# veeresht/CommPy

Measured on AMD Instinct MI355X. Metric: decoded info-bits/s at fixed Eb/N0 (Viterbi K=7 r=1/2, 1024b); BER match, higher is better.
Workload: dtype f64

## Files before the change

commpy_amd/csrc/viterbi_cw.hip:

```cpp
#include "cpx_internal.h"
#include "cpx_math.h"
#include "viterbi_cw_asm.h"
#ifndef CPX_GEN_GB
#define CPX_GEN_GB 2
#endif

#include <atomic>
#include <cstdlib>
#include <cstring>
#include <mutex>
#include <type_traits>

using namespace cpx;

namespace {

template <int LGS, unsigned G0, unsigned G1>
struct SrCode {
    static constexpr int S = 1 << LGS;
    static constexpr int parity(unsigned v) { return __builtin_popcount(v) & 1; }
    static constexpr int code(int s, int j) {
        const unsigned p = (unsigned)(((s << 1) & (S - 1)) | j), b = (unsigned)(s >> (LGS - 1));
        const unsigned reg = (b << LGS) | p;
        return (parity(reg & G0) << 1) | parity(reg & G1);
    }
};

template <int LGS>
constexpr int rotl(int s, int r) {
    r %= LGS;
    return r == 0 ? s : (((s << r) | (s >> (LGS - r))) & ((1 << LGS) - 1));
}

__device__ __forceinline__ double vmin(double a, double b) {
    double r;
    asm("v_min_f64 %0, %1, %2" : "=v"(r) : "v"(a), "v"(b));
    return r;
}

__device__ __forceinline__ double acs_min(unsigned &acc, double x, double y) {
    double r;
    asm("v_cmp_lt_f64 vcc, %3, %2\n\tv_addc_co_u32 %1, vcc, %1, %1, vcc\n\tv_min_f64 %0, %2, %3"
        : "=&v"(r), "+v"(acc) : "v"(x), "v"(y) : "vcc");
    return r;
}
__device__ __forceinline__ double acs_min_first(unsigned &acc, double x, double y) {
    double r;
    asm("v_cmp_lt_f64 vcc, %3, %2\n\tv_cndmask_b32 %1, 0, 1, vcc\n\tv_min_f64 %0, %2, %3"
        : "=&v"(r), "=&v"(acc) : "v"(x), "v"(y) : "vcc");
    return r;
}

__device__ __forceinline__ double acs_select(unsigned &acc, double x, double y) {
    int rlo, rhi;
    asm("v_cmp_lt_f64 vcc, %4, %3\n\tv_cndmask_b32 %0, %5, %7, vcc\n\tv_cndmask_b32 %1, %6, %8, vcc\n\t"
        "v_addc_co_u32 %2, vcc, %2, %2, vcc"
        : "=&v"(rlo), "=&v"(rhi), "+v"(acc)
        : "v"(x), "v"(y), "v"(__double2loint(x)), "v"(__double2hiint(x)), "v"(__double2loint(y)), "v"(__double2hiint(y))
        : "vcc");
    return __hiloint2double(rhi, rlo);
}

struct CwParams {
    const double *coded;
    unsigned long long *dec;
    unsigned char *best;
    uint8_t *bits;
    uint8_t *nanflags;
    int64_t B, len, L, T, Lk, Tp;
    int type, tb;
    unsigned goff[4];
};

__device__ __forceinline__ void nan_or(unsigned long long &mask, double r0, double r1) {
#ifdef CPX_AB_NO_NAN_DETECT
    (void)mask; (void)r0; (void)r1;
    return;
#endif
    asm("v_cmp_u_f64 vcc, %1, %2\n\ts_or_b64 %0, %0, vcc" : "+s"(mask) : "v"(r0), "v"(r1) : "vcc", "scc");
}

__device__ __forceinline__ void bit_metrics_cw(int type, double r, double &m0, double &m1) {
    if (type == CPX_VIT_HARD) {
        long long ri = (long long)r;
        m0 = (double)(ri ^ 0ll);
        m1 = (double)(ri ^ 1ll);
    } else if (type == CPX_VIT_SOFT) {
        double nll0 = fast_log<false>(exp(r) + 1.0);
        m0 = nll0;
        m1 = nll0 - r;
    } else {
        double d0 = r - (-1.0), d1 = r - 1.0;
        m0 = d0 * d0;
        m1 = d1 * d1;
    }
}

__device__ __forceinline__ double clip500(double r) {
    double c;
    asm("v_max_f64 %0, %1, %2\n\tv_min_f64 %0, %0, %3" : "=&v"(c) : "v"(r), "s"(-500.0), "s"(500.0));
    return c;
}
__device__ __forceinline__ void soft_metrics_lean(double r, double &m0, double &m1) {
    const double nll0 = fast_log<false, false, true>(exp_pm500(r) + 1.0);
    m0 = nll0;
    m1 = nll0 - r;
}

template <int LGS>
__device__ __forceinline__ unsigned tb_hop(unsigned long long w, unsigned st) {
    const unsigned hi = (unsigned)((w << (st & ((1u << LGS) - 1u))) >> 32);
    return __builtin_amdgcn_alignbit(st, hi, 31);
}

struct NoHook {
    template <int P> __device__ __forceinline__ void at() const {}
};

template <int LGS, unsigned G0, unsigned G1, int TYPE, int R, bool LEAN = false, class Hook = NoHook>
__device__ __forceinline__ void cw_step(double (&pm)[1 << LGS], double r0, double r1, unsigned long long &word, int &best,
                                        const Hook &hook = Hook(), unsigned char *bml = nullptr, const unsigned *gidx = nullptr) {
    constexpr int type = TYPE;
    using C = SrCode<LGS, G0, G1>;
    constexpr bool GEN = G0 == 0 && G1 == 0;
    constexpr int S = 1 << LGS, H = S / 2;
    double m00, m01, m10, m11;
    if constexpr (LEAN && TYPE == CPX_VIT_SOFT) {
        r0 = clip500(r0);
        r1 = clip500(r1);
        soft_metrics_lean(r0, m00, m01);
        soft_metrics_lean(r1, m10, m11);
    } else {
        if (type == CPX_VIT_SOFT) {
            r0 = fmin(fmax(r0, -500.0), 500.0);
            r1 = fmin(fmax(r1, -500.0), 500.0);
        }
        bit_metrics_cw(type, r0, m00, m01);
        bit_metrics_cw(type, r1, m10, m11);
    }
    double bmv[4];
    if constexpr (LEAN) {
        bmv[0] = m00 + m10; bmv[1] = m00 + m11;
        bmv[2] = m01 + m10; bmv[3] = m01 + m11;
    } else {
        bmv[0] = (0.0 + m00) + m10; bmv[1] = (0.0 + m00) + m11;
        bmv[2] = (0.0 + m01) + m10; bmv[3] = (0.0 + m01) + m11;
    }
    unsigned da = 0, db = 0;
    hook.template at<0>();
    auto butterfly = [&](int j, double m_a0, double m_a1, double m_b0, double m_b1) {
        const int x = rotl<LGS>(2 * j, R), y = rotl<LGS>(2 * j + 1, R);
        const double a = pm[x], b = pm[y];
        const double a0 = a + m_a0, a1 = b + m_a1;
        const double b0 = a + m_b0, b1 = b + m_b1;
        if (TYPE == CPX_VIT_UNQUANTIZED) {
            pm[x] = acs_select(da, a0, a1);
            pm[y] = acs_select(db, b0, b1);
        } else if (j == 0) {
            pm[x] = acs_min_first(da, a0, a1);
            pm[y] = acs_min_first(db, b0, b1);
        } else {
            pm[x] = acs_min(da, a0, a1);
            pm[y] = acs_min(db, b0, b1);
        }
    };
    if constexpr (GEN) {
        typedef double cpx_d4 __attribute__((ext_vector_type(4)));
        const cpx_d4 tab = {bmv[0], bmv[1], bmv[2], bmv[3]}, rtab = {bmv[3], bmv[2], bmv[1], bmv[0]};
        asm volatile("s_set_gpr_idx_on 0, 1" ::: "memory", "m0");
        auto acs_pair = [&](int j, double a0, double a1, double b0, double b1) {
            const int x = rotl<LGS>(2 * j, R), y = rotl<LGS>(2 * j + 1, R);
            if (TYPE == CPX_VIT_UNQUANTIZED) {
                pm[x] = acs_select(da, a0, a1);
                pm[y] = acs_select(db, b0, b1);
            } else {
                pm[x] = acs_min(da, a0, a1);
                pm[y] = acs_min(db, b0, b1);
            }
        };
        if constexpr (H >= 4 && TYPE != CPX_VIT_UNQUANTIZED) {
#pragma unroll
            for (int j = 0; j < H; j += 2) {
                if (j == H / 2) hook.template at<1>();
                const int x0 = rotl<LGS>(2 * j, R), y0 = rotl<LGS>(2 * j + 1, R), x1 = rotl<LGS>(2 * j + 2, R), y1 = rotl<LGS>(2 * j + 3, R);
                const double a = pm[x0], b = pm[y0], c = pm[x1], d = pm[y1];
                double a0, a1, b0, b1, c0, c1, d0, d1;
                asm volatile("s_set_gpr_idx_idx %[i0]\n\t"
                             "v_add_f64 %[a0], v[248:249], %[a]\n\t"
                             "v_add_f64 %[b1], v[248:249], %[b]\n\t"
                             "v_add_f64 %[a1], v[240:241], %[b]\n\t"
                             "v_add_f64 %[b0], v[240:241], %[a]\n\t"
                             "s_set_gpr_idx_idx %[i1]\n\t"
                             "v_add_f64 %[c0], v[248:249], %[c]\n\t"
                             "v_add_f64 %[d1], v[248:249], %[d]\n\t"
                             "v_add_f64 %[c1], v[240:241], %[d]\n\t"
                             "v_add_f64 %[d0], v[240:241], %[c]\n\t"
                             "s_set_gpr_idx_idx 0\n\t"
                             "v_cmp_lt_f64 vcc, %[a1], %[a0]\n\tv_addc_co_u32 %[da], vcc, %[da], %[da], vcc\n\tv_min_f64 %[a0], %[a0], %[a1]\n\t"
                             "v_cmp_lt_f64 vcc, %[b1], %[b0]\n\tv_addc_co_u32 %[db], vcc, %[db], %[db], vcc\n\tv_min_f64 %[b0], %[b0], %[b1]\n\t"
                             "v_cmp_lt_f64 vcc, %[c1], %[c0]\n\tv_addc_co_u32 %[da], vcc, %[da], %[da], vcc\n\tv_min_f64 %[c0], %[c0], %[c1]\n\t"
                             "v_cmp_lt_f64 vcc, %[d1], %[d0]\n\tv_addc_co_u32 %[db], vcc, %[db], %[db], vcc\n\tv_min_f64 %[d0], %[d0], %[d1]"
                             : [a0] "=&v"(a0), [a1] "=&v"(a1), [b0] "=&v"(b0), [b1] "=&v"(b1), [c0] "=&v"(c0), [c1] "=&v"(c1),
                               [d0] "=&v"(d0), [d1] "=&v"(d1), [da] "+v"(da), [db] "+v"(db)
                             : [i0] "s"(gidx[j]), [i1] "s"(gidx[j + 1]), [a] "v"(a), [b] "v"(b), [c] "v"(c), [d] "v"(d),
                               "{v[248:255]}"(tab), "{v[240:247]}"(rtab)
                             : "vcc", "m0");
                pm[x0] = a0; pm[y0] = b0;
                pm[x1] = c0; pm[y1] = d0;
            }
        } else {
#pragma unroll
            for (int j = 0; j < H; j++) {
                if (j == H / 2) hook.template at<1>();
                const double a = pm[rotl<LGS>(2 * j, R)], b = pm[rotl<LGS>(2 * j + 1, R)];
                double a0, a1, b0, b1;
                asm volatile("s_set_gpr_idx_idx %[ic]\n\t"
                             "v_add_f64 %[a0], v[248:249], %[a]\n\t"
                             "v_add_f64 %[b1], v[248:249], %[b]\n\t"
                             "v_add_f64 %[a1], v[240:241], %[b]\n\t"
                             "v_add_f64 %[b0], v[240:241], %[a]\n\t"
                             "s_set_gpr_idx_idx 0"
                             : [a0] "=&v"(a0), [a1] "=&v"(a1), [b0] "=&v"(b0), [b1] "=&v"(b1)
                             : [ic] "s"(gidx[j]), [a] "v"(a), [b] "v"(b), "{v[248:255]}"(tab), "{v[240:247]}"(rtab)
                             : "m0");
                acs_pair(j, a0, a1, b0, b1);
            }
        }
        asm volatile("s_set_gpr_idx_off" ::: "memory", "m0");
    } else {
#pragma unroll
        for (int j = 0; j < H; j++) {
            if (j == H / 2) hook.template at<1>();
            butterfly(j, bmv[C::code(j, 0)], bmv[C::code(j, 1)], bmv[C::code(j + H, 0)], bmv[C::code(j + H, 1)]);
        }
    }
    hook.template at<2>();
    int bst = 0;
    constexpr bool ARGMIN32 = LEAN && S == 64 && TYPE == CPX_VIT_SOFT && !GEN;
    unsigned long long tie = ~0ull;
    if constexpr (ARGMIN32) {
#define CPX_HI(s) "v"(__double2hiint(pm[rotl<LGS>((s), R + 1)]))
#define CPX_COL(i) CPX_HI(i), CPX_HI((i) + 8), CPX_HI((i) + 16), CPX_HI((i) + 24), CPX_HI((i) + 32), CPX_HI((i) + 40), CPX_HI((i) + 48), CPX_HI((i) + 56)
#define CPX_ROW(j) CPX_HI(8 * (j)), CPX_HI(8 * (j) + 1), CPX_HI(8 * (j) + 2), CPX_HI(8 * (j) + 3), CPX_HI(8 * (j) + 4), CPX_HI(8 * (j) + 5), CPX_HI(8 * (j) + 6), CPX_HI(8 * (j) + 7)
        unsigned q0, q1, q2, q3, q4, q5, q6, q7, m, w;
        asm(CPX_COL_BLOCK3 : "=&v"(q0), "=&v"(q1), "=&v"(q2) : CPX_COL(0), CPX_COL(1), CPX_COL(2));
        asm(CPX_COL_BLOCK3 : "=&v"(q3), "=&v"(q4), "=&v"(q5) : CPX_COL(3), CPX_COL(4), CPX_COL(5));
        asm(CPX_COL_BLOCK_LAST : "=&v"(q6), "=&v"(q7), "=&v"(m), "=&v"(w) : "v"(q0), "v"(q1), "v"(q2), "v"(q3), "v"(q4), "v"(q5), CPX_COL(6), CPX_COL(7)
            : "vcc");
        hook.template at<3>();
        unsigned r0_, r1_, r2_;
        asm(CPX_ROW_BLOCK3 : "+v"(w), "=&v"(r0_), "=&v"(r1_), "=&v"(r2_) : "v"(m), CPX_ROW(7), CPX_ROW(6), CPX_ROW(5) : "vcc");
        asm(CPX_ROW_BLOCK3 : "+v"(w), "=&v"(r0_), "=&v"(r1_), "=&v"(r2_) : "v"(m), CPX_ROW(4), CPX_ROW(3), CPX_ROW(2) : "vcc");
        asm(CPX_ROW_BLOCK_LAST : "+v"(w), "=&v"(r0_), "=&v"(r1_), "=&v"(bst), "=&s"(tie) : "v"(m), CPX_ROW(1), CPX_ROW(0) : "vcc");
#undef CPX_ROW
#undef CPX_COL
#undef CPX_HI
    }
    if (__builtin_expect(tie != 0, !ARGMIN32)) {
        double m0 = pm[0], m1 = pm[1 % S], m2 = pm[2 % S], m3 = pm[3 % S];
        if constexpr (S == 64) {
#define CPX_V4(a) "v"(pm[a]), "v"(pm[(a) + 1]), "v"(pm[(a) + 2]), "v"(pm[(a) + 3])
            asm(CPX_MIN_BLOCK24 : "+v"(m0), "+v"(m1), "+v"(m2), "+v"(m3)
                : CPX_V4(4), CPX_V4(8), CPX_V4(12), CPX_V4(16), CPX_V4(20), CPX_V4(24));
            asm(CPX_MIN_BLOCK24 : "+v"(m0), "+v"(m1), "+v"(m2), "+v"(m3)
                : CPX_V4(28), CPX_V4(32), CPX_V4(36), CPX_V4(40), CPX_V4(44), CPX_V4(48));
            asm(CPX_MIN_BLOCK12 : "+v"(m0), "+v"(m1), "+v"(m2), "+v"(m3) : CPX_V4(52), CPX_V4(56), CPX_V4(60));
#undef CPX_V4
        } else {
#pragma unroll
            for (int s = 4; s < S; s += 4) {
                m0 = vmin(m0, pm[s]); m1 = vmin(m1, pm[s + 1]); m2 = vmin(m2, pm[s + 2]); m3 = vmin(m3, pm[s + 3]);
            }
        }
        const double mn = vmin(vmin(m0, m1), vmin(m2, m3));
        if constexpr (!ARGMIN32) hook.template at<3>();
        if constexpr (S == 64) {
            unsigned long long k0, k1, k2, k3;
#define CPX_S4(a) "v"(pm[rotl<LGS>((a), R + 1)]), "v"(pm[rotl<LGS>((a) - 1, R + 1)]), "v"(pm[rotl<LGS>((a) - 2, R + 1)]), "v"(pm[rotl<LGS>((a) - 3, R + 1)])
            asm(CPX_SCAN_BLOCK0 : "+v"(bst), "=&s"(k0), "=&s"(k1), "=&s"(k2), "=&s"(k3)
                : "v"(mn), CPX_S4(63), CPX_S4(59), CPX_S4(55), CPX_S4(51), CPX_S4(47), CPX_S4(43));
            asm(CPX_SCAN_BLOCK1 : "+v"(bst), "=&s"(k0), "=&s"(k1), "=&s"(k2), "=&s"(k3)
                : "v"(mn), CPX_S4(39), CPX_S4(35), CPX_S4(31), CPX_S4(27), CPX_S4(23), CPX_S4(19));
            asm(CPX_SCAN_BLOCK2 : "+v"(bst), "=&s"(k0), "=&s"(k1), "=&s"(k2), "=&s"(k3)
                : "v"(mn), CPX_S4(15), CPX_S4(11), CPX_S4(7), CPX_S4(3));
#undef CPX_S4
        } else if constexpr (S % 4 == 0) {
#pragma unroll
            for (int s = S - 4; s >= 0; s -= 4) {
                unsigned long long k0, k1, k2, k3;
                asm("v_cmp_eq_f64 %1, %5, %9\n\tv_cmp_eq_f64 %2, %6, %9\n\tv_cmp_eq_f64 %3, %7, %9\n\tv_cmp_eq_f64 %4, %8, %9\n\t"
                    "v_cndmask_b32 %0, %0, %10, %1\n\tv_cndmask_b32 %0, %0, %11, %2\n\tv_cndmask_b32 %0, %0, %12, %3\n\t"
                    "v_cndmask_b32 %0, %0, %13, %4"
                    : "+v"(bst), "=&s"(k0), "=&s"(k1), "=&s"(k2), "=&s"(k3)
                    : "v"(pm[rotl<LGS>(s + 3, R + 1)]), "v"(pm[rotl<LGS>(s + 2, R + 1)]), "v"(pm[rotl<LGS>(s + 1, R + 1)]),
                      "v"(pm[rotl<LGS>(s, R + 1)]), "v"(mn), "n"(s + 3), "n"(s + 2), "n"(s + 1), "n"(s));
            }
        } else {
#pragma unroll
            for (int s = S - 1; s >= 0; s--) bst = (pm[rotl<LGS>(s, R + 1)] == mn) ? s : bst;
        }
    }
    word = ((unsigned long long)da << (64 - H)) | ((unsigned long long)db << (64 - S));
    best = bst;
}

__device__ __forceinline__ float acs_min_f32(unsigned &acc, float x, float y) {
    float r;
    asm("v_cmp_lt_f32 vcc, %3, %2\n\tv_addc_co_u32 %1, vcc, %1, %1, vcc\n\tv_min_f32 %0, %2, %3"
        : "=&v"(r), "+v"(acc) : "v"(x), "v"(y) : "vcc");
    return r;
}
__device__ __forceinline__ float vmin3_f32(float a, float b, float c) {
    float r;
    asm("v_min3_f32 %0, %1, %2, %3" : "=v"(r) : "v"(a), "v"(b), "v"(c));
    return r;
}
__device__ __forceinline__ void bit_metrics_f32(int type, double r, float &m0, float &m1) {
    if (type == CPX_VIT_HARD) {
        const long long ri = (long long)r;
        m0 = (float)(ri ^ 0ll);
        m1 = (float)(ri ^ 1ll);
    } else if (type == CPX_VIT_SOFT) {
        m0 = 0.0f;
        m1 = -(float)r;
    } else {
        const float x = (float)r, d0 = x + 1.0f, d1 = x - 1.0f;
        m0 = d0 * d0;
        m1 = d1 * d1;
    }
}

template <int LGS, unsigned G0, unsigned G1, int TYPE, int R, bool LEAN = false, class Hook = NoHook>
__device__ __forceinline__ void cw_step(float (&pm)[1 << LGS], double r0, double r1, unsigned long long &word, int &best,
                                        const Hook &hook = Hook(), unsigned char * = nullptr, const unsigned * = nullptr) {
    using C = SrCode<LGS, G0, G1>;
    constexpr int S = 1 << LGS, H = S / 2;
    if (TYPE == CPX_VIT_SOFT) {
        r0 = fmin(fmax(r0, -500.0), 500.0);
        r1 = fmin(fmax(r1, -500.0), 500.0);
    }
    float m00, m01, m10, m11;
    bit_metrics_f32(TYPE, r0, m00, m01);
    bit_metrics_f32(TYPE, r1, m10, m11);
    float bmv[4];
    bmv[0] = (0.0f + m00) + m10; bmv[1] = (0.0f + m00) + m11;
    bmv[2] = (0.0f + m01) + m10; bmv[3] = (0.0f + m01) + m11;
    unsigned da = 0, db = 0;
    hook.template at<0>();
#pragma unroll
    for (int j = 0; j < H; j++) {
        if (j == H / 2) hook.template at<1>();
        const int x = rotl<LGS>(2 * j, R), y = rotl<LGS>(2 * j + 1, R);
        const float a = pm[x], b = pm[y];
        const float a0 = a + bmv[C::code(j, 0)], a1 = b + bmv[C::code(j, 1)];
        const float b0 = a + bmv[C::code(j + H, 0)], b1 = b + bmv[C::code(j + H, 1)];
        pm[x] = acs_min_f32(da, a0, a1);
        pm[y] = acs_min_f32(db, b0, b1);
    }
    hook.template at<2>();
    float mn;
    if constexpr (S >= 8 && S % 8 == 0) {
        float m0 = pm[0], m1 = pm[1], m2 = pm[2], m3 = pm[3];
#pragma unroll
        for (int s = 4; s + 8 <= S; s += 8) {
            m0 = vmin3_f32(m0, pm[s], pm[s + 1]); m1 = vmin3_f32(m1, pm[s + 2], pm[s + 3]);
            m2 = vmin3_f32(m2, pm[s + 4], pm[s + 5]); m3 = vmin3_f32(m3, pm[s + 6], pm[s + 7]);
        }
        m0 = vmin3_f32(m0, pm[S - 4], pm[S - 3]);
        m1 = vmin3_f32(m1, pm[S - 2], pm[S - 1]);
        mn = fminf(vmin3_f32(m0, m1, m2), m3);
    } else {
        mn = pm[0];
#pragma unroll
        for (int s = 1; s < S; s++) mn = fminf(mn, pm[s]);
    }
    hook.template at<3>();
    int bst = 0;
    if constexpr (S % 4 == 0) {
#pragma unroll
        for (int s = S - 4; s >= 0; s -= 4) {
            unsigned long long k0, k1, k2, k3;
            asm("v_cmp_eq_f32 %1, %5, %9\n\tv_cmp_eq_f32 %2, %6, %9\n\tv_cmp_eq_f32 %3, %7, %9\n\tv_cmp_eq_f32 %4, %8, %9\n\t"
                "v_cndmask_b32 %0, %0, %10, %1\n\tv_cndmask_b32 %0, %0, %11, %2\n\tv_cndmask_b32 %0, %0, %12, %3\n\t"
                "v_cndmask_b32 %0, %0, %13, %4"
                : "+v"(bst), "=&s"(k0), "=&s"(k1), "=&s"(k2), "=&s"(k3)
                : "v"(pm[rotl<LGS>(s + 3, R + 1)]), "v"(pm[rotl<LGS>(s + 2, R + 1)]), "v"(pm[rotl<LGS>(s + 1, R + 1)]),
                  "v"(pm[rotl<LGS>(s, R + 1)]), "v"(mn), "n"(s + 3), "n"(s + 2), "n"(s + 1), "n"(s));
        }
    } else {
#pragma unroll
        for (int s = S - 1; s >= 0; s--) bst = (pm[rotl<LGS>(s, R + 1)] == mn) ? s : bst;
    }
    word = ((unsigned long long)da << (64 - H)) | ((unsigned long long)db << (64 - S));
    best = bst;
}

constexpr int ACS_WAVES = 4;

template <int LGS, unsigned G0, unsigned G1, int TYPE>
__global__ __launch_bounds__(64 * ACS_WAVES) void viterbi_cw_acs_kernel(CwParams p) {
    constexpr int S = 1 << LGS;
    const int lane = threadIdx.x & 63;
    const int64_t grp = (int64_t)blockIdx.x * ACS_WAVES + (threadIdx.x >> 6);
    const int64_t cw = grp * 64 + lane;
    if (grp * 64 >= p.B) return;
    const bool valid = cw < p.B;
    const double *x = p.coded + (valid ? cw : 0) * p.len;
    unsigned long long *dec = p.dec + grp * p.Tp * 64 + lane;
    unsigned char *best = p.best + grp * p.Tp * 64 + lane;

    double pm[S];
#pragma unroll
    for (int s = 0; s < S; s++) pm[s] = (s == 0) ? 0.0 : __builtin_huge_val();

    const double pad = (TYPE == CPX_VIT_UNQUANTIZED) ? -1.0 : 0.0;
    const int T = (int)p.T, tmax = (int)((p.Lk < p.T) ? p.Lk : p.T);
    auto load = [&](int t) {
        const int tc = (t < tmax) ? t : tmax;
        return *reinterpret_cast<const double2 *>(x + (int64_t)(tc - 1) * 2);
    };
    double2 cur[LGS], nxt[LGS];
#pragma unroll
    for (int u = 0; u < LGS; u++) cur[u] = load(1 + u);
    unsigned long long nanmask = 0;
    for (int t = 1; t <= T; t += LGS) {
#pragma unroll
        for (int u = 0; u < LGS; u++) nxt[u] = load(t + LGS + u);
#pragma unroll
        for (int u = 0; u < LGS; u++) {
            const bool have = t + u <= tmax;
            cur[u].x = have ? cur[u].x : pad;
            cur[u].y = have ? cur[u].y : pad;
        }
        unsigned long long *d = dec + (int64_t)(t - 1) * 64;
        unsigned char *b = best + (int64_t)(t - 1) * 64;
        auto one = [&](auto rtag, const double2 &v) {
            constexpr int R = decltype(rtag)::value;
            unsigned long long word;
            int bst;
            if constexpr (TYPE == CPX_VIT_SOFT) nan_or(nanmask, v.x, v.y);
            cw_step<LGS, G0, G1, TYPE, R>(pm, v.x, v.y, word, bst);
            d[R * 64] = word;
            b[R * 64] = (unsigned char)bst;
        };
        if constexpr (LGS >= 1) one(std::integral_constant<int, 0>{}, cur[0]);
        if constexpr (LGS >= 2) one(std::integral_constant<int, 1>{}, cur[1 % LGS]);
        if constexpr (LGS >= 3) one(std::integral_constant<int, 2>{}, cur[2 % LGS]);
        if constexpr (LGS >= 4) one(std::integral_constant<int, 3>{}, cur[3 % LGS]);
        if constexpr (LGS >= 5) one(std::integral_constant<int, 4>{}, cur[4 % LGS]);
        if constexpr (LGS >= 6) one(std::integral_constant<int, 5>{}, cur[5 % LGS]);
#pragma unroll
        for (int u = 0; u < LGS; u++) cur[u] = nxt[u];
    }
    static_assert(LGS == 6, "viterbi_cw_acs_kernel writes per-codeword NaN flags: valid for 64-state trellises only (items of one codeword)");
    if constexpr (TYPE == CPX_VIT_SOFT)
        if (valid) p.nanflags[cw] = (uint8_t)((nanmask >> lane) & 1ull);
}

constexpr int FR_RING = 32, FR_CHUNK = 96, FR_OBPAD = 100;
constexpr int FR_RING_DEEP = 64;

template <int RING, bool MIR> constexpr int fused_slots() { return MIR ? 2 * RING + 2 : RING + 1; }
template <int RING, bool MIR, bool GEN = false>
constexpr size_t fused_wave_lds() {
    return (size_t)fused_slots<RING, MIR>() * 64 * 8 + (size_t)64 * FR_OBPAD;
}

constexpr int WAIT_LGKM0 = 0xC07F;
template <int LGS, int H, bool RT = false, int RING = FR_RING, bool MIR = true, bool LATE = false>
struct WalkHook {
    static constexpr int NH = RT ? (H > LGS - 1 ? H - (LGS - 1) : 0) : H;
    static constexpr int NB = 4, PER = (NH + NB - 1) / NB;
    const unsigned long long *pw;
    int q;
    mutable unsigned st;
    int he, sh;
    mutable unsigned long long buf[LATE ? (NH > 0 ? NH : 1) : (PER > 0 ? PER : 1)];
    __device__ __forceinline__ unsigned long long word(int h) const {
        return MIR ? pw[(RING - h) * 64] : pw[((q - h) & (RING - 1)) * 64];
    }
    template <int B> __device__ __forceinline__ void issue() const {
#pragma unroll
        for (int i = 0; i < PER; i++)
            if (B * PER + i < NH) buf[LATE ? B * PER + i : i] = word(B * PER + i);
    }
    template <int B> __device__ __forceinline__ void hops() const {
#pragma unroll
        for (int i = 0; i < PER; i++)
            if (B * PER + i < NH) {
                const unsigned nx = tb_hop<LGS>(buf[LATE ? B * PER + i : i], st);
                st = (!RT || B * PER + i < he) ? nx : st;
            }
    }
    template <int P> __device__ __forceinline__ void at() const {
        __builtin_amdgcn_sched_barrier(0);
        if constexpr (!LATE && P > 0) hops<P - 1>();
        issue<P>();
        __builtin_amdgcn_sched_barrier(0);
    }
    __device__ __forceinline__ void finish() const {
        __builtin_amdgcn_sched_barrier(0);
        if constexpr (LATE) {
            if constexpr (NH > 0) {
                __builtin_amdgcn_s_waitcnt(WAIT_LGKM0);
                asm volatile("" : "+v"(st));
            }
            hops<0>(); hops<1>(); hops<2>(); hops<3>();
        } else {
            hops<NB - 1>();
        }
        __builtin_amdgcn_sched_barrier(0);
    }
    __device__ __forceinline__ unsigned bit() const { return (st >> (RT ? sh : LGS - 1)) & 1u; }
};

template <int LGS, unsigned G0, unsigned G1, int TYPE, int HT, bool RT = false, class F = double, int RING = FR_RING, bool MIR = true>
__global__ __launch_bounds__(64 * ACS_WAVES) void viterbi_cw_fused_kernel(CwParams p) {
    constexpr int S = 1 << LGS, FR_GROUPS = FR_CHUNK / LGS, CHUNK = FR_GROUPS * LGS;
    static_assert(HT >= 0 && HT + 1 <= RING && (RING & (RING - 1)) == 0 && CHUNK + 1 <= FR_OBPAD, "ring / tile too small");
    const int H = RT ? p.tb - 2 : HT;
    constexpr bool GEN = G0 == 0 && G1 == 0;
#ifdef CPX_VIT_SPEC_LG
    __shared__ __attribute__((aligned(16))) unsigned char smem[ACS_WAVES * fused_wave_lds<RING, MIR, GEN>()];
#else
    extern __shared__ __attribute__((aligned(16))) unsigned char smem[];
#endif
    const int lane = threadIdx.x & 63, wv = threadIdx.x >> 6;
    const int64_t grp = (int64_t)blockIdx.x * ACS_WAVES + wv;
    const int64_t cw = grp * 64 + lane;
    if (grp * 64 >= p.B) return;
    if constexpr (LGS == 6 && !MIR && !GEN && RING == FR_RING) __builtin_amdgcn_s_setprio(3);
    const bool valid = cw < p.B;
    const double *x = p.coded + (valid ? cw : 0) * p.len;
    static_assert(!GEN || (!MIR && std::is_same<F, double>::value), "table-driven codes: unmirrored ring, float64");
    unsigned long long *ring = reinterpret_cast<unsigned long long *>(smem + (size_t)wv * fused_wave_lds<RING, MIR, GEN>());
    unsigned char *obuf = reinterpret_cast<unsigned char *>(ring + fused_slots<RING, MIR>() * 64);
    unsigned long long *mycol = ring + lane;
    unsigned char *myrow = obuf + lane * FR_OBPAD;

    F pm[S];
#pragma unroll
    for (int s = 0; s < S; s++) pm[s] = (s == 0) ? (F)0.0 : (F)__builtin_huge_val();
    unsigned gidx[GEN ? S / 2 : 1];
#pragma unroll
    for (int j = 0; j < (GEN ? S / 2 : 1); j++) gidx[j] = GEN ? __builtin_amdgcn_ubfe(p.goff[j >> 3], 4 * (j & 7), 4) : 0u;

    const double pad = (TYPE == CPX_VIT_UNQUANTIZED) ? -1.0 : 0.0;
    const int T = (int)p.T, tmax = (int)((p.Lk < p.T) ? p.Lk : p.T);
    auto load = [&](int t) {
        const int tc = (t < tmax) ? t : tmax;
        return *reinterpret_cast<const double2 *>(x + (int64_t)(tc - 1) * 2);
    };
    double2 cur[LGS];
#pragma unroll
    for (int u = 0; u < LGS; u++) cur[u] = load(1 + u);
    int best_T = 0;
    unsigned long long nanmask = 0;
    constexpr bool LATE = LGS == 6 && TYPE == CPX_VIT_SOFT && !GEN && std::is_same<F, double>::value;
    WalkHook<LGS, HT, RT, RING, MIR, LATE> walk;
    walk.pw = mycol;
    walk.q = 0;
    walk.st = 0;
    walk.he = H > LGS - 1 ? H - (LGS - 1) : 0;
    walk.sh = H > LGS - 1 ? 0 : LGS - 1 - H;

    const int so_max = (int)((p.L < (int64_t)(T - H)) ? p.L : (int64_t)(T - H));
    auto flush = [&](int tc0, int n) {
        asm volatile("s_waitcnt lgkmcnt(0)" ::: "memory");
        const int64_t cwb = grp * 64;
        const int ncw = (int)((p.B - cwb < 64) ? (p.B - cwb) : 64);
        const int so0 = tc0 - 1 - H;
        const int lo = so0 >= 1 ? 0 : 1 - so0;
        const int hi = (so_max - so0 + 1 < n) ? so_max - so0 + 1 : n;
        if (lo < hi) {
            const bool w0 = lane >= lo && lane < hi, w1 = lane + 64 >= lo && lane + 64 < hi;
            const unsigned o0 = (unsigned)(lane - lo), o1 = o0 + 64u;
            const int l1 = (lane + 64 < FR_OBPAD) ? lane + 64 : FR_OBPAD - 1;
            unsigned char *row = p.bits + cwb * p.L + (so0 + lo - 1);
            for (int c0 = 0; c0 < ncw; c0 += 8) {
                unsigned char v[8][2];
#pragma unroll
                for (int u = 0; u < 8; u++) {
                    v[u][0] = obuf[(c0 + u) * FR_OBPAD + lane];
                    v[u][1] = obuf[(c0 + u) * FR_OBPAD + l1];
                }
                if (c0 + 8 <= ncw) {
                    if (w0) {
#pragma unroll
                        for (int u = 0; u < 8; u++) row[(int64_t)u * p.L + o0] = v[u][0];
                    }
                    if (w1) {
#pragma unroll
                        for (int u = 0; u < 8; u++) row[(int64_t)u * p.L + o1] = v[u][1];
                    }
                } else {
#pragma unroll
                    for (int u = 0; u < 8; u++)
                        if (c0 + u < ncw) {
                            if (w0) row[(int64_t)u * p.L + o0] = v[u][0];
                            if (w1) row[(int64_t)u * p.L + o1] = v[u][1];
                        }
                }
                row += 8 * p.L;
            }
        }
        asm volatile("s_waitcnt lgkmcnt(0)" ::: "memory");
    };

    auto group = [&](auto ftag, const int t, unsigned char *tile) __attribute__((always_inline)) {
        constexpr bool FAST = decltype(ftag)::value;
        double2 nxt[LGS];
        const double2 *xt = reinterpret_cast<const double2 *>(x) + (t - 1);
#pragma unroll
        for (int u = 0; u < LGS; u++) nxt[u] = FAST ? xt[LGS + u] : load(t + LGS + u);
        auto one = [&](auto rtag) {
            constexpr int R = decltype(rtag)::value;
            const int tt = t + R;
            const bool have = FAST || tt <= tmax;
            const double r0 = have ? cur[R].x : pad, r1 = have ? cur[R].y : pad;
            unsigned long long word;
            int bst;
            if constexpr (TYPE == CPX_VIT_SOFT) nan_or(nanmask, cur[R].x, cur[R].y);
            cw_step<LGS, G0, G1, TYPE, R, true>(pm, r0, r1, word, bst, walk, nullptr, gidx);
            walk.finish();
            tile[R] = (unsigned char)walk.bit();
            const bool live = FAST || tt <= T;
            const int q = tt & (RING - 1);
            unsigned long long *wb = mycol + q * 64;
            if constexpr (MIR) {
                unsigned long long *w0 = live ? wb : mycol + (2 * RING) * 64;
                unsigned long long *w1 = live ? wb + RING * 64 : mycol + (2 * RING + 1) * 64;
                *w0 = word;
                *w1 = word;
                walk.pw = wb;
            } else {
                unsigned long long *w0 = live ? wb : mycol + RING * 64;
                *w0 = word;
                walk.q = q;
            }
            if constexpr (!FAST) best_T = (tt == T) ? bst : best_T;
            walk.st = (unsigned)bst;
        };
        if constexpr (LGS >= 1) one(std::integral_constant<int, 0>{});
        if constexpr (LGS >= 2) one(std::integral_constant<int, 1 % LGS>{});
        if constexpr (LGS >= 3) one(std::integral_constant<int, 2 % LGS>{});
        if constexpr (LGS >= 4) one(std::integral_constant<int, 3 % LGS>{});
        if constexpr (LGS >= 5) one(std::integral_constant<int, 4 % LGS>{});
        if constexpr (LGS >= 6) one(std::integral_constant<int, 5 % LGS>{});
#pragma unroll
        for (int u = 0; u < LGS; u++) cur[u] = nxt[u];
    };

    for (int tc0 = 1; tc0 <= T; tc0 += CHUNK) {
        const int left = (T - tc0) / LGS + 1;
        const int ngroups = left < FR_GROUPS ? left : FR_GROUPS;
        const int room = tmax - tc0 - (2 * LGS - 1);
        const int nfast = room < 0 ? 0 : (room / LGS + 1 < ngroups ? room / LGS + 1 : ngroups);
        int t = tc0;
        unsigned char *tile = myrow;
        for (int g = 0; g < nfast; g++, t += LGS, tile += LGS) group(std::true_type{}, t, tile);
        for (int g = nfast; g < ngroups; g++, t += LGS, tile += LGS) group(std::false_type{}, t, tile);
        int n = ngroups * LGS;
        if (tc0 + CHUNK > T) {
            unsigned st = walk.st;
            for (int h = 0; h < H; h++) st = tb_hop<LGS>(walk.word(h), st);
            myrow[n] = (unsigned char)((st >> (LGS - 1)) & 1u);
            n++;
        }
        flush(tc0, n);
    }
    if constexpr (TYPE == CPX_VIT_SOFT)
    {
            constexpr int CPI = 64 / S;
            const int64_t item = grp * (64 / CPI) + lane;
            if (lane < 64 / CPI && item * CPI < p.B)
                p.nanflags[item] = (uint8_t)(((nanmask >> (lane * CPI)) & (CPI == 64 ? ~0ull : ((1ull << CPI) - 1ull))) != 0);
        }
    if (valid) {
        const int qT = T & (RING - 1);
        unsigned st = (unsigned)best_T;
        for (int h = 0; h < H; h++) {
            const int so = T - h;
            if (so < 1) break;
            if (so - 1 < p.L) p.bits[cw * p.L + so - 1] = (uint8_t)((st >> (LGS - 1)) & 1u);
            st = tb_hop<LGS>(mycol[((qT - h) & (RING - 1)) * 64], st);
        }
    }
}

constexpr int TB_THREADS = 512, TB_WAVES = TB_THREADS / 64, TB_STRIDE = 65;

template <int LGS>
__global__ __launch_bounds__(TB_THREADS) void viterbi_cw_tb_kernel(CwParams p) {
    (void)LGS;
    extern __shared__ __attribute__((aligned(16))) unsigned char smem[];
    const int H = p.tb - 2, rows = 64 + H;
    unsigned long long *win = reinterpret_cast<unsigned long long *>(smem);
    unsigned char *bwin = reinterpret_cast<unsigned char *>(win + (size_t)rows * TB_STRIDE);
    const int lane = threadIdx.x & 63, w = threadIdx.x >> 6;
    const int64_t grp = blockIdx.x;
    const unsigned long long *dec = p.dec + grp * p.Tp * 64;
    const unsigned char *best = p.best + grp * p.Tp * 64;
    for (int64_t base = 1; base <= p.T; base += 64) {
        int64_t need = base + 63 + H;
        if (need > p.T) need = p.T;
        __syncthreads();
        for (int64_t tt = base + w; tt <= need; tt += TB_WAVES) {
            win[(tt - base) * TB_STRIDE + lane] = dec[(tt - 1) * 64 + lane];
            bwin[(tt - base) * 64 + lane] = best[(tt - 1) * 64 + lane];
        }
        __syncthreads();
        const int64_t so = base + lane;
        const bool full = base + 63 + H <= p.T;
        int64_t t0 = so + H;
        if (t0 > p.T) t0 = p.T;
        for (int c0 = w; c0 < 64; c0 += 2 * TB_WAVES) {
            const int c1 = c0 + TB_WAVES;
            unsigned st0 = 0, st1 = 0;
            if (so <= p.T) {
                st0 = bwin[(t0 - base) * 64 + c0];
                st1 = bwin[(t0 - base) * 64 + c1];
            }
            int idx = (lane + H) * TB_STRIDE;
            if (full) {
#pragma unroll 4
                for (int h = 0; h < H; h++) {
                    st0 = tb_hop<LGS>(win[idx + c0], st0);
                    st1 = tb_hop<LGS>(win[idx + c1], st1);
                    idx -= TB_STRIDE;
                }
            } else {
                for (int h = 0; h < H; h++) {
                    const bool go = so + H - h <= p.T;
                    const unsigned n0 = tb_hop<LGS>(win[idx + c0], st0), n1 = tb_hop<LGS>(win[idx + c1], st1);
                    st0 = go ? n0 : st0;
                    st1 = go ? n1 : st1;
                    idx -= TB_STRIDE;
                }
            }
            const int64_t pos = so - 1;
            if (so <= p.T && pos < p.L) {
                const int64_t cwa = grp * 64 + c0, cwb = grp * 64 + c1;
                if (cwa < p.B) p.bits[cwa * p.L + pos] = (uint8_t)((st0 >> (LGS - 1)) & 1u);
                if (cwb < p.B) p.bits[cwb * p.L + pos] = (uint8_t)((st1 >> (LGS - 1)) & 1u);
            }
        }
    }
}

template <int RING_, bool MIR_, int HOPS_>
struct Flavour {
    static constexpr int RING = RING_, HOPS = HOPS_;
    static constexpr bool MIR = MIR_;
};
template <int LGS> constexpr int fused_tb() { return 5 * LGS; }
template <int LGS> constexpr int fused_tb_deep() { return 8 * LGS; }
template <int LGS> using Mirrored32 = Flavour<FR_RING, true, fused_tb<LGS>() - 2>;
template <int LGS> using Deep64 = Flavour<FR_RING_DEEP, false, fused_tb_deep<LGS>() - 2>;
template <int LGS> using Lean32 = Flavour<FR_RING, false, fused_tb<LGS>() - 2>;
template <int LGS> using Small = Flavour<(fused_tb<LGS>() - 1 <= 16 ? 16 : 32), false, fused_tb<LGS>() - 2>;

template <class FL, int LGS, unsigned G0, unsigned G1, int TYPE, bool RT, class F>
bool launch_fused_kernel(const CwParams &p, hipStream_t st) {
    auto *fn = viterbi_cw_fused_kernel<LGS, G0, G1, TYPE, FL::HOPS, RT, F, FL::RING, FL::MIR>;
    constexpr size_t lds = ACS_WAVES * fused_wave_lds<FL::RING, FL::MIR, G0 == 0 && G1 == 0>();
    if (lds > 64 * 1024) {
        static bool raised[64] = {};
        static std::mutex raised_mu;
        int dev = 0;
        if (hipGetDevice(&dev) != hipSuccess || dev < 0 || dev >= 64) return false;
        std::lock_guard<std::mutex> lk(raised_mu);
        if (!raised[dev]) {
            if (hipFuncSetAttribute((const void *)fn, hipFuncAttributeMaxDynamicSharedMemorySize, (int)lds) != hipSuccess) {
                (void)hipGetLastError();
                return false;
            }
            raised[dev] = true;
        }
    }
    const unsigned groups = (unsigned)((p.B + 63) / 64), blocks = (groups + ACS_WAVES - 1) / ACS_WAVES;
    hipLaunchKernelGGL(fn, dim3(blocks), dim3(64 * ACS_WAVES), lds, st, p);
    return true;
}

template <class FL, int LGS, unsigned G0, unsigned G1, class F, bool RT>
bool launch_fused_rt(const CwParams &p, hipStream_t st) {
    if (p.type == CPX_VIT_HARD) return launch_fused_kernel<FL, LGS, G0, G1, CPX_VIT_HARD, RT, F>(p, st);
    if (p.type == CPX_VIT_SOFT) return launch_fused_kernel<FL, LGS, G0, G1, CPX_VIT_SOFT, RT, F>(p, st);
    return launch_fused_kernel<FL, LGS, G0, G1, CPX_VIT_UNQUANTIZED, RT, F>(p, st);
}
template <class FL, int LGS, unsigned G0, unsigned G1, class F = double>
bool launch_fused(const CwParams &p, hipStream_t st) {
    return p.tb != FL::HOPS + 2 ? launch_fused_rt<FL, LGS, G0, G1, F, true>(p, st) : launch_fused_rt<FL, LGS, G0, G1, F, false>(p, st);
}

template <int LGS, unsigned G0, unsigned G1>
void launch_two_kernels(const CwParams &p, size_t tb_lds, hipStream_t st) {
    const unsigned groups = (unsigned)((p.B + 63) / 64), ablocks = (groups + ACS_WAVES - 1) / ACS_WAVES;
    const dim3 ab(64 * ACS_WAVES);
    if (p.type == CPX_VIT_HARD) hipLaunchKernelGGL((viterbi_cw_acs_kernel<LGS, G0, G1, CPX_VIT_HARD>), dim3(ablocks), ab, 0, st, p);
    else if (p.type == CPX_VIT_SOFT) hipLaunchKernelGGL((viterbi_cw_acs_kernel<LGS, G0, G1, CPX_VIT_SOFT>), dim3(ablocks), ab, 0, st, p);
    else hipLaunchKernelGGL((viterbi_cw_acs_kernel<LGS, G0, G1, CPX_VIT_UNQUANTIZED>), dim3(ablocks), ab, 0, st, p);
    hipLaunchKernelGGL((viterbi_cw_tb_kernel<LGS>), dim3(groups), dim3(TB_THREADS), tb_lds, st, p);
}

}

#ifdef CPX_VIT_SPEC_LG
namespace {
constexpr int SPEC_LG = CPX_VIT_SPEC_LG;
constexpr int SPEC_RING = SPEC_LG == 6 ? FR_RING : (5 * SPEC_LG - 1 <= 16 ? 16 : 32);
constexpr bool SPEC_MIR = SPEC_LG == 6;
#define CPX_SPEC(TYPE, RT)                                                                                                  \
    template __global__ void viterbi_cw_fused_kernel<SPEC_LG, CPX_VIT_SPEC_G0, CPX_VIT_SPEC_G1, TYPE, 5 * SPEC_LG - 2, RT, double, \
                                                     SPEC_RING, SPEC_MIR>(CwParams);
CPX_SPEC(CPX_VIT_HARD, false) CPX_SPEC(CPX_VIT_HARD, true) CPX_SPEC(CPX_VIT_SOFT, false) CPX_SPEC(CPX_VIT_SOFT, true)
CPX_SPEC(CPX_VIT_UNQUANTIZED, false) CPX_SPEC(CPX_VIT_UNQUANTIZED, true)
#undef CPX_SPEC
}
#else

namespace {

struct Pair { int lg; unsigned g0, g1; };
constexpr Pair BUILTIN_PAIRS[] = {
    {6, 0155u, 0117u},
    {6, 0117u, 0155u},
    {6, 0133u, 0171u},
    {6, 0171u, 0133u},
    {6, 0120u, 0152u},
    {2, 05u, 07u},
    {4, 031u, 027u},
};
constexpr int N_BUILTIN = sizeof(BUILTIN_PAIRS) / sizeof(BUILTIN_PAIRS[0]);

int builtin_index(const TrellisClass &c) {
    if (c.linear_half)
        for (int i = 0; i < N_BUILTIN; i++)
            if (BUILTIN_PAIRS[i].lg == c.lgS && BUILTIN_PAIRS[i].g0 == c.g0 && BUILTIN_PAIRS[i].g1 == c.g1) return i;
    return -1;
}

const char *type_name(int type) { return type == CPX_VIT_HARD ? "hard" : type == CPX_VIT_SOFT ? "soft" : "unquantized"; }

struct CwCall {
    CwParams p;
    Scratch *sc;
    hipStream_t st;
    size_t tb_lds;
    int64_t groups;
    bool lean_ring, two_kernels, f32;
};

CwResult done(CwFlavour f, const char *form) {
    if (hipGetLastError() == hipSuccess) return {true, CPX_OK, f};
    set_error("viterbi (%scodeword path): launch failed", form);
    return {true, CPX_EHIP, f};
}

template <int LG, unsigned GA, unsigned GB>
CwResult run_builtin(CwCall &c) {
    CwParams &p = c.p;
    const int tb = p.tb, type = p.type;
    if constexpr (LG == 6) {
        if (c.lean_ring && type == CPX_VIT_SOFT && tb == fused_tb<LG>() && !c.two_kernels && !c.f32 &&
            launch_fused_kernel<Lean32<LG>, LG, GA, GB, CPX_VIT_SOFT, false, double>(p, c.st)) {
            const CwResult r = done(CwFlavour::lean, "fused ");
            note_kernel("viterbi_cw_fused_kernel<%d,0%o,0%o,%s,%d,ring stored once>", LG, GA, GB, type_name(type), fused_tb<LG>() - 2);
            return r;
        }
        const bool deep = tb > fused_tb<LG>();
        if (tb >= 2 && tb <= fused_tb_deep<LG>() && !c.two_kernels &&
            (deep ? launch_fused_rt<Deep64<LG>, LG, GA, GB, double, true>(p, c.st)
                  : c.f32 ? launch_fused<Mirrored32<LG>, LG, GA, GB, float>(p, c.st) : launch_fused<Mirrored32<LG>, LG, GA, GB, double>(p, c.st))) {
            const CwResult r = done(deep ? CwFlavour::deep : CwFlavour::mirrored, "fused ");
            note_kernel("viterbi_cw_fused_kernel<%d,0%o,0%o,%s,%d%s%s>", LG, GA, GB, type_name(type),
                        (deep ? fused_tb_deep<LG>() : fused_tb<LG>()) - 2,
                        deep ? ",runtime hops,64-slot ring" : tb == fused_tb<LG>() ? "" : ",runtime hops", (c.f32 && !deep) ? ",f32" : "");
            return r;
        }
        p.Tp = (p.T + LG - 1) / LG * LG;
        if (int rc = c.sc->get(c.st, Slot::state, sizeof(unsigned long long) * (size_t)(c.groups * p.Tp * 64), &p.dec)) return {true, rc, CwFlavour::two_kernels};
        if (int rc = c.sc->get(c.st, Slot::state2, (size_t)(c.groups * p.Tp * 64), &p.best)) return {true, rc, CwFlavour::two_kernels};
        launch_two_kernels<LG, GA, GB>(p, c.tb_lds, c.st);
        const CwResult r = done(CwFlavour::two_kernels, "");
        note_kernel("viterbi_cw_acs_kernel<%d,0%o,0%o,%s> + viterbi_cw_tb_kernel<%d>", LG, GA, GB, type_name(type), LG);
        return r;
    } else {
        if (tb >= 2 && tb <= fused_tb<LG>() && !c.two_kernels && !c.f32 && launch_fused<Small<LG>, LG, GA, GB>(p, c.st)) {
            const CwResult r = done(CwFlavour::small, "small fused ");
            note_kernel("viterbi_cw_fused_kernel<%d,0%o,0%o,%s,%d,small ring%s>", LG, GA, GB, type_name(type), fused_tb<LG>() - 2,
                        tb == fused_tb<LG>() ? "" : ",runtime hops");
            return r;
        }
        return {};
    }
}
template <int I = 0>
CwResult run_builtin_at(int i, CwCall &c) {
    if constexpr (I < N_BUILTIN) {
        constexpr Pair P = BUILTIN_PAIRS[I];
        return i == I ? run_builtin<P.lg, P.g0, P.g1>(c) : run_builtin_at<I + 1>(i, c);
    } else {
        return {};
    }
}

template <int LG = 6>
CwResult run_table(int lg, CwCall &c) {
    if constexpr (LG >= 2) {
        if (lg != LG) return run_table<LG - 1>(lg, c);
        if (!launch_fused<Small<LG>, LG, 0u, 0u>(c.p, c.st)) return {};
        const CwResult r = done(CwFlavour::table, "table-driven ");
        note_kernel("viterbi_cw_fused_kernel<%d,table-driven,%s,%d%s>", LG, type_name(c.p.type), fused_tb<LG>() - 2,
                    c.p.tb == fused_tb<LG>() ? "" : ",runtime hops");
        return r;
    } else {
        return {};
    }
}

}

namespace cpx {

CwResult viterbi_codeword_path(const cpx_trellis *t, const double *d_coded, int64_t B, int64_t len, int64_t L, int64_t T,
                               int tb, int type, uint8_t *d_bits, uint8_t *nanflags, Scratch &sc, hipStream_t st, bool any_batch_size,
                               bool lean_ring) {
    const int pf = viterbi_path_flags();
    if (pf & 1) return {};
    const bool forced = (pf & 2) || any_batch_size, strict = pf & 4;
    auto reject = [&](const char *why) -> CwResult {
        if (!strict) return {};
        set_error("viterbi (codeword path): %s", why);
        return {true, CPX_ELIMIT, CwFlavour::none};
    };
    if (!forced && !viterbi_round_pays(B, viterbi_round())) return {};
    const TrellisClass &k = t->cls;
    if (t->I != 2 || t->k != 1 || t->n != 2 || T < 1) return reject("needs a rate-1/2, k = 1 trellis");
    if ((len & 1) || ((uintptr_t)d_coded & 15)) return reject("rows must be 16-byte aligned");
    CwCall c;
    c.sc = &sc;
    c.st = st;
    c.tb_lds = (size_t)(64 + tb - 2) * (TB_STRIDE * 8 + 64);
    if (c.tb_lds > 64 * 1024) return reject("traceback window exceeds 64 KiB of LDS");
    c.groups = (B + 63) / 64;
    if (c.groups >= (1ll << 31) || T >= (1ll << 31) - 64) return reject("batch too large / block too long");
    CwParams &p = c.p;
    p.coded = d_coded; p.bits = d_bits; p.B = B; p.len = len; p.L = L; p.T = T; p.Lk = L;
    p.type = type; p.tb = tb; p.nanflags = nanflags;
    if (type == CPX_VIT_SOFT && !nanflags) return reject("'soft' needs the NaN flag array");
    c.lean_ring = lean_ring;
    c.two_kernels = pf & 8;
    c.f32 = precision_fast() && T < (1ll << 22);
    if (const CwResult r = run_builtin_at(builtin_index(k), c); r.handled) return r;
    const bool plain = tb >= 2 && !c.two_kernels && !c.f32;
    if (t->spec_mod && plain && tb <= 5 * t->spec_lg) {
        const bool rt = tb != 5 * t->spec_lg;
        hipFunction_t fn = t->spec_fn[type][rt ? 1 : 0];
        const unsigned groups32 = (unsigned)c.groups, blocks = (groups32 + ACS_WAVES - 1) / ACS_WAVES;
        void *args[] = {(void *)&p};
        if (hipModuleLaunchKernel(fn, blocks, 1, 1, 64 * ACS_WAVES, 1, 1, 0, st, args, nullptr) != hipSuccess) {
            (void)hipGetLastError();
            set_error("viterbi (per-pair code object): launch failed");
            return {true, CPX_EHIP, CwFlavour::code_object};
        }
        note_kernel("viterbi_cw_fused_kernel<%d,0%o,0%o,%s,%d%s> (code object of this pair)", t->spec_lg, t->spec_g0, t->spec_g1,
                    type_name(type), 5 * t->spec_lg - 2, rt ? ",runtime hops" : "");
        return {true, CPX_OK, CwFlavour::code_object};
    }
    if (k.end_tap && plain && tb <= 5 * k.lgS) {
        memcpy(p.goff, k.goff, sizeof(p.goff));
        if (const CwResult r = run_table(k.lgS, c); r.handled) return r;
    }
    return reject("no instantiation for this trellis");
}

}

extern "C" int cpx_viterbi_set_path(const char *mode) { return cpx::set_mode(cpx::Switch::viterbi_path, mode); }

extern "C" int cpx_trellis_viterbi_spec_query(const cpx_trellis *t, int *lg, unsigned *g0, unsigned *g1) {
    CPX_REQUIRE(t && lg && g0 && g1, CPX_EINVAL, "cpx_trellis_viterbi_spec_query: null pointer");
    *lg = 0; *g0 = 0; *g1 = 0;
    const cpx::TrellisClass &k = t->cls;
    if (!k.end_tap || !k.linear_half || builtin_index(k) >= 0 || t->spec_mod) return CPX_OK;
    *lg = k.lgS; *g0 = k.g0; *g1 = k.g1;
    return CPX_OK;
}

extern "C" int cpx_trellis_attach_viterbi_code(cpx_trellis *t, const void *image, size_t bytes) {
    CPX_REQUIRE(t && image && bytes >= 64, CPX_EINVAL, "cpx_trellis_attach_viterbi_code: null / empty image");
    if (int rcd = cpx::check_handle_device(t->device, "attach_viterbi_code")) return rcd;
    CPX_REQUIRE(!t->spec_mod, CPX_EINVAL, "cpx_trellis_attach_viterbi_code: the trellis already has a code object");
    CPX_REQUIRE(t->cls.linear_half, CPX_EINVAL,
                "cpx_trellis_attach_viterbi_code: not a rate-1/2 shift-register code of 4 .. 64 states");
    const int lg = t->cls.lgS;
    const unsigned g0 = t->cls.g0, g1 = t->cls.g1;
    hipModule_t mod = nullptr;
    if (hipModuleLoadData(&mod, image) != hipSuccess) {
        (void)hipGetLastError();
        cpx::set_error("cpx_trellis_attach_viterbi_code: hipModuleLoadData refused the image");
        return CPX_EHIP;
    }
    const int ring = lg == 6 ? FR_RING : (5 * lg - 1 <= 16 ? 16 : 32);
    hipFunction_t fn[3][2];
    for (int type = 0; type < 3; type++)
        for (int rt = 0; rt < 2; rt++) {
            char name[200];
            snprintf(name, sizeof(name), "_ZN12_GLOBAL__N_123viterbi_cw_fused_kernelILi%dELj%uELj%uELi%dELi%dELb%dEdLi%dELb%dEEEvNS_8CwParamsE",
                     lg, g0, g1, type, 5 * lg - 2, rt, ring, lg == 6 ? 1 : 0);
            if (hipModuleGetFunction(&fn[type][rt], mod, name) != hipSuccess) {
                (void)hipGetLastError();
                (void)hipModuleUnload(mod);
                cpx::set_error("cpx_trellis_attach_viterbi_code: the image has no kernel %s (compiled for other generators, or from other sources)", name);
                return CPX_EINVAL;
            }
        }
    memcpy(t->spec_fn, fn, sizeof(fn));
    t->spec_lg = lg; t->spec_g0 = g0; t->spec_g1 = g1;
    t->spec_mod = mod;
    return CPX_OK;
}

extern "C" int cpx_trellis_has_viterbi_code(const cpx_trellis *t) { return (t && t->spec_mod) ? 1 : 0; }

extern "C" int cpx_trellis_detach_viterbi_code(cpx_trellis *t) {
    CPX_REQUIRE(t, CPX_EINVAL, "cpx_trellis_detach_viterbi_code: null trellis");
    if (t->spec_mod) {
        (void)hipDeviceSynchronize();
        (void)hipModuleUnload(t->spec_mod);
        t->spec_mod = nullptr;
        t->spec_lg = 0;
    }
    return CPX_OK;
}
#endif
```

Measured before the change: 52.61 billion.

## Batch six traceback walks per group into one burst of shared word loads

Adds a WalkBurst hook that, once per group of LGS trellis steps, loads the window of decision words once and advances six traceback walks together. Each walk no longer issues its own loads and hops after every ACS step. Per-step LDS traffic and latency stalls should fall, and the interleaved walks give more independent work. In exchange it needs more registers for the word window and walk states, which could lower occupancy or cause spills, and it is enabled only for the K=7 soft double mirrored path.

```diff
diff --git a/commpy_amd/csrc/viterbi_cw.hip b/commpy_amd/csrc/viterbi_cw.hip
--- a/commpy_amd/csrc/viterbi_cw.hip
+++ b/commpy_amd/csrc/viterbi_cw.hip
@@ -514,6 +514,39 @@
     __device__ __forceinline__ unsigned bit() const { return (st >> (RT ? sh : LGS - 1)) & 1u; }
 };
 
+template <int LGS, int NHE, int RING, bool RT>
+struct WalkBurst {
+    static constexpr int NW = NHE + LGS - 1;
+    static constexpr int NB = 4, PER = 2 * ((NW + 2 * NB - 1) / (2 * NB));
+    const unsigned long long *pb;
+    int he, sh;
+    mutable unsigned st[LGS];
+    mutable unsigned long long w[NW];
+    template <int P> __device__ __forceinline__ void at() const {
+        __builtin_amdgcn_sched_barrier(0);
+#pragma unroll
+        for (int i = 0; i < PER; i++)
+            if (P * PER + i < NW) w[P * PER + i] = pb[(RING - (P * PER + i)) * 64];
+        __builtin_amdgcn_sched_barrier(0);
+    }
+    __device__ __forceinline__ void finish() const {
+        static_assert(LGS == 6, "the walk states are named one by one below");
+        __builtin_amdgcn_sched_barrier(0);
+        __builtin_amdgcn_s_waitcnt(WAIT_LGKM0);
+        asm volatile("" : "+v"(st[0]), "+v"(st[1]), "+v"(st[2]), "+v"(st[3]), "+v"(st[4]), "+v"(st[5]));
+#pragma unroll
+        for (int h = 0; h < NHE; h++) {
+#pragma unroll
+            for (int k = 0; k < LGS; k++) {
+                const unsigned nx = tb_hop<LGS>(w[LGS - 1 - k + h], st[k]);
+                st[k] = (!RT || h < he) ? nx : st[k];
+            }
+        }
+        __builtin_amdgcn_sched_barrier(0);
+    }
+    __device__ __forceinline__ unsigned bit(int k) const { return (st[k] >> (RT ? sh : 0)) & 1u; }
+};
+
 template <int LGS, unsigned G0, unsigned G1, int TYPE, int HT, bool RT = false, class F = double, int RING = FR_RING, bool MIR = true>
 __global__ __launch_bounds__(64 * ACS_WAVES) void viterbi_cw_fused_kernel(CwParams p) {
     constexpr int S = 1 << LGS, FR_GROUPS = FR_CHUNK / LGS, CHUNK = FR_GROUPS * LGS;
@@ -563,6 +596,15 @@
     walk.st = 0;
     walk.he = H > LGS - 1 ? H - (LGS - 1) : 0;
     walk.sh = H > LGS - 1 ? 0 : LGS - 1 - H;
+    constexpr bool BURST = LATE && MIR && HT > LGS - 1;
+    constexpr int NHE = BURST ? HT - (LGS - 1) : 1;
+    static_assert(!BURST || NHE + LGS <= RING, "ring too small for the words of LGS walks at once");
+    WalkBurst<LGS, NHE, RING, RT> burst;
+    burst.pb = mycol;
+    burst.he = walk.he;
+    burst.sh = walk.sh;
+#pragma unroll
+    for (int k = 0; k < LGS; k++) burst.st[k] = 0;
 
     const int so_max = (int)((p.L < (int64_t)(T - H)) ? p.L : (int64_t)(T - H));
     auto flush = [&](int tc0, int n) {
@@ -621,9 +663,19 @@
             unsigned long long word;
             int bst;
             if constexpr (TYPE == CPX_VIT_SOFT) nan_or(nanmask, cur[R].x, cur[R].y);
+            if constexpr (BURST && R == LGS - 1) {
+                burst.pb = mycol + ((tt - 1) & (RING - 1)) * 64;
+                cw_step<LGS, G0, G1, TYPE, R, true>(pm, r0, r1, word, bst, burst, nullptr, gidx);
+                burst.finish();
+#pragma unroll
+                for (int k = 0; k < LGS; k++) tile[k] = (unsigned char)burst.bit(k);
+            } else if constexpr (BURST) {
+                cw_step<LGS, G0, G1, TYPE, R, true>(pm, r0, r1, word, bst, NoHook(), nullptr, gidx);
+            } else {
             cw_step<LGS, G0, G1, TYPE, R, true>(pm, r0, r1, word, bst, walk, nullptr, gidx);
             walk.finish();
             tile[R] = (unsigned char)walk.bit();
+            }
             const bool live = FAST || tt <= T;
             const int q = tt & (RING - 1);
             unsigned long long *wb = mycol + q * 64;
@@ -640,6 +692,7 @@
             }
             if constexpr (!FAST) best_T = (tt == T) ? bst : best_T;
             walk.st = (unsigned)bst;
+            if constexpr (BURST) burst.st[(R + 1) % LGS] = (unsigned)bst;
         };
         if constexpr (LGS >= 1) one(std::integral_constant<int, 0>{});
         if constexpr (LGS >= 2) one(std::integral_constant<int, 1 % LGS>{});
```

Result: faster. 54.20 billion, median of 6 (+3.0%).
